# pujariaditya/WaveVerify

Measured on AMD Instinct MI355X. Metric: clips/sec embed+detect, 1s@16kHz bs=256, higher is better.
Workload: dtype f32; 1 GPU; embed_detect: 256 clips x 1 s @ 16 kHz per GPU (BASELINE.json configs[1]), seeded random weights; batch_per_gpu=256, global_batch=256, clip_samples=16000, parallelism=dp1 (independent clip shards, no data-path collective)

## Files before the change

### waveverify_amd/csrc/wv_k1.hip

```cpp
#include <algorithm>
#include <atomic>
#include <cstdlib>
#include <string>
#include <type_traits>

#include "wv_dev.h"

namespace wv {

typedef const __attribute__((address_space(1))) void* gptr_t;
typedef __attribute__((address_space(3))) void* lptr_t;

__device__ __attribute__((aligned(16))) float g_zero16[4] = {0.f, 0.f, 0.f, 0.f};

__device__ __forceinline__ float dpp_next(float v) {
    return __builtin_bit_cast(float, __builtin_amdgcn_update_dpp(0, __builtin_bit_cast(int, v), 0x130, 0xf, 0xf, true));
}

template <int NT_, int BKC_, int BM_ = 128>
struct K1 {
    static constexpr int NT = NT_, BN = 32 * NT_, BKC = BKC_, KQ = BKC_ / 4, BM = BM_, WM = BM_ / 32, NTHREADS = 64 * WM;
    static constexpr int A4 = KQ * BM;
    static constexpr int B4 = BKC * BN / 4;
    static constexpr int STAGE4 = A4 + B4;
    static constexpr int A_PIECES = A4 / 64, B_PIECES = B4 / 64;
    static constexpr int A_PER = (A_PIECES + WM - 1) / WM, B_PER_DMA = (B_PIECES + WM - 1) / WM;
    static constexpr int CG = BN / 4;
    static constexpr int HLD = BN + 4;
    static constexpr int NBT = (BKC / 2) * CG;
    static constexpr int B_PER = (NBT + NTHREADS - 1) / NTHREADS;
    static_assert(A4 % 64 == 0 && B4 % 64 == 0 && NTHREADS % CG == 0 && 64 % CG == 0, "staging maps");
};

template <int NT> struct NVec;
template <> struct NVec<4> { typedef f32x4 type; };
template <> struct NVec<2> { typedef f32x2 type; };

constexpr int OOB_VOFF = 0x40000000;

template <class C>
struct DmaRows {
    const float* src; size_t ld; int K; int rbase;
    __device__ __forceinline__ void init(const float* Xb, int K_, int Tin, int ti0, int wave, int lane) {
        const int col = ti0 + 4 * (lane % C::CG);
        rbase = lane / C::CG;
        const bool inr = col >= 0 && col + 3 < Tin;
        src = inr ? Xb + col : g_zero16;
        ld = inr ? (size_t)Tin : 0;
        K = K_;
        (void)wave;
    }
    __device__ __forceinline__ void init_flat(const float* X, int K_, int Tin, int B, int Tv, int pad, long long g0, int lane) {
        const long long g = g0 + 4 * (lane % C::CG);
        const int b = (int)(g / Tv), t = (int)(g - (long long)b * Tv) - pad;
        rbase = lane / C::CG;
        const bool inr = b < B && t >= 0;
        src = inr ? X + (size_t)b * K_ * Tin + t : g_zero16;
        ld = inr ? (size_t)Tin : 0;
        K = K_;
    }
    __device__ __forceinline__ void issue(int c, f32x4* Bst, int wave) const {
#pragma unroll
        for (int i = 0; i < C::B_PER_DMA; ++i) {
            const int pi = wave + i * C::WM;
            if (C::B_PIECES % C::WM == 0 || pi < C::B_PIECES) {
                const int k = min(c * C::BKC + pi * (64 / C::CG) + rbase, K - 1);
                __builtin_amdgcn_global_load_lds((gptr_t)(src + (size_t)k * ld), (lptr_t)(Bst + pi * 64), 16, 0, 0);
            }
        }
    }
};

template <class C>
struct DmaA {
    __amdgpu_buffer_rsrc_t rsrc;
    int voff[C::A_PER];
    int chunk_bytes;
    __device__ __forceinline__ void init(const f32x4* wq, int Mp, int m0, int nchunks, int wave, int lane) {
        rsrc = __builtin_amdgcn_make_buffer_rsrc(const_cast<f32x4*>(wq + m0), 0, (nchunks * C::KQ * Mp - m0) * 16, 0x00020000);
        chunk_bytes = C::KQ * Mp * 16;
#pragma unroll
        for (int i = 0; i < C::A_PER; ++i) {
            const int idx = (wave + i * C::WM) * 64 + lane;
            voff[i] = ((idx / C::BM) * Mp + idx % C::BM) * 16;
        }
    }
    __device__ __forceinline__ void issue(int c, f32x4* Ast, int wave) const {
        const int soff = c * chunk_bytes;
#pragma unroll
        for (int i = 0; i < C::A_PER; ++i) {
            const int pi = wave + i * C::WM;
            if (C::A_PIECES % C::WM == 0 || pi < C::A_PIECES) {
                const int vo = voff[i];
                __builtin_amdgcn_raw_ptr_buffer_load_lds(rsrc, (lptr_t)(Ast + pi * 64), 16, vo, soff, 0, 0);
            }
        }
    }
};

template <class C, int EPI, int RES>
struct K1Epi {
    static constexpr int NT = C::NT, HLD = C::HLD;
    static constexpr int NTAP = EPI == 0 ? 5 : (EPI == 2 ? 4 : (EPI == 4 ? 8 : 16));
    static constexpr int WLD = EPI == 0 ? 8 : NTAP + 4;
    static constexpr int TABLE_FLOATS = C::BM * WLD;
    static constexpr bool HASR = RES == 1 || RES == 2 || RES == 5;
    static constexpr bool RAWH = RES == 4 || RES == 5;
    static constexpr int RP = HASR ? 4 : 0;
    typedef typename NVec<NT>::type ovec;
    int M, m0, b, to0, lane, wave, half, q, o, to;
    bool act_lane, vec;
    const float* Rb; float* Yb; float* Ab; float* Wl;
    const float* Rb2; float* Hb; float* Sb;
    int voff0, nrec;
    float fgam, fbet;

    __device__ __forceinline__ int row_of(int r) const { return 32 * wave + (r & 3) + 8 * (r >> 2) + 4 * half; }
    __device__ __forceinline__ ovec load_res(const PwDwArgs& p, int r) const {
        ovec v;
#pragma unroll
        for (int e = 0; e < NT; ++e) v[e] = 0.f;
        const int gm = m0 + row_of(r);
        if (act_lane && gm < M) {
            const float* rp = Rb + (size_t)gm * p.Tout + to;
            if (vec) v = *reinterpret_cast<const ovec*>(rp);
            else {
#pragma unroll
                for (int e = 0; e < NT; ++e)
                    if (o + e < p.tto && to + e < p.Tout) v[e] = rp[e];
            }
        }
        return v;
    }
    __device__ __forceinline__ void store(const PwDwArgs& p, int gm, const float (&y)[NT]) const {
        const size_t yo = (size_t)gm * p.Tout + to;
        if (Yb) {
            if (vec) { ovec v; _Pragma("unroll") for (int e = 0; e < NT; ++e) v[e] = y[e]; *reinterpret_cast<ovec*>(Yb + yo) = v; }
            else {
#pragma unroll
                for (int e = 0; e < NT; ++e)
                    if (o + e < p.tto && to + e < p.Tout) Yb[yo + e] = y[e];
            }
        }
        if (Ab) {
            float a[NT];
#pragma unroll
            for (int e = 0; e < NT; ++e) a[e] = elu1(y[e] * p.act_scale);
            if (vec) { ovec v; _Pragma("unroll") for (int e = 0; e < NT; ++e) v[e] = a[e]; *reinterpret_cast<ovec*>(Ab + yo) = v; }
            else {
#pragma unroll
                for (int e = 0; e < NT; ++e)
                    if (o + e < p.tto && to + e < p.Tout) Ab[yo + e] = a[e];
            }
        }
    }
    __device__ __forceinline__ void begin(const PwDwArgs& p, float* table, int m0_, int b_, int to0_, long long gflat = 0) {
        M = p.pw.M; m0 = m0_; b = b_; to0 = to0_;
        const int tid = threadIdx.x;
        lane = tid & 63;
        wave = __builtin_amdgcn_readfirstlane(tid >> 6);
        half = lane >> 5; q = lane & 31;
        Wl = table;
        const size_t bo = (size_t)b * M * p.Tout;
        Yb = p.Y ? p.Y + bo : nullptr;
        Ab = p.Yact ? p.Yact + bo : nullptr;
        Rb = (HASR && p.resid) ? p.resid + bo : nullptr;
        Rb2 = (RES == 2 && p.resid2) ? p.resid2 + bo : nullptr;
        Hb = (RAWH && p.Yraw) ? p.Yraw + bo : nullptr;
        Sb = (RES == 5 && p.Ysum) ? p.Ysum + bo : nullptr;
        o = NT * q; to = to0 + o;
        act_lane = o < p.tto && to < p.Tout;
        vec = act_lane && to + NT - 1 < p.Tout && o + NT - 1 < p.tto && (p.Tout % NT) == 0;
        nrec = M * p.Tout * 4;
        voff0 = act_lane ? ((m0 + 32 * wave + 4 * half) * p.Tout + to) * 4 : 0x7f000000;
        if (EPI == 0 && p.flat) {
            const long long gc = gflat + p.pad + o;
            const int bo2 = (int)(gc / p.Tv), t = (int)(gc - (long long)bo2 * p.Tv) - p.pad;
            const bool ok = o < p.tto && bo2 < p.B && t >= 0;
            Yb = p.Y; Ab = p.Yact; Rb = HASR ? p.resid : nullptr; Rb2 = RES == 2 ? p.resid2 : nullptr; Hb = RAWH ? p.Yraw : nullptr; Sb = RES == 5 ? p.Ysum : nullptr;
            nrec = (int)((long long)p.B * M * p.Tout * 4);
            voff0 = ok ? (int)((((long long)bo2 * M + m0 + 32 * wave + 4 * half) * p.Tout + t) * 4) : (int)0x80000000u;
        }
        if (EPI == 8 && p.flat) {
            const int TvO = p.Tv >> 3;
            const long long go = gflat / 8 + (q >> 1);
            const int bo2 = (int)(go / TvO), n = (int)(go - (long long)bo2 * TvO);
            const bool ok = (q & 1) == 0 && (q >> 1) < p.tto && bo2 < p.B && n < p.Tout;
            Yb = p.Y; Ab = p.Yact;
            nrec = (int)((long long)p.B * M * p.Tout * 4);
            voff0 = ok ? (int)((((long long)bo2 * M + m0 + 32 * wave + 4 * half) * p.Tout + n) * 4) : (int)0x80000000u;
            fgam = 1.f; fbet = 0.f;
            if (p.film) {
                const float* fl = p.film + (size_t)min(bo2, p.B - 1) * p.film_stride + 2 * (m0 / (M / p.bands));
                fgam = fl[0]; fbet = fl[1];
            }
        }
        const bool lane_film = EPI == 8 && p.flat;
        const int bw = p.film ? (M / p.bands) : 1;
        const float* filmb = (p.film && !lane_film) ? p.film + (size_t)b * p.film_stride : nullptr;
        for (int m = tid; m < C::BM; m += C::NTHREADS) {
            const int gm = m0 + m;
            float* row = Wl + m * WLD;
#pragma unroll
            for (int i = 0; i < NTAP; ++i) row[i] = (gm < M && i < p.ks) ? p.dw_w[(size_t)gm * p.ks + i] : 0.f;
            float gam = 1.f, bet = 0.f;
            if (filmb && gm < M) { const int band = gm / bw; gam = filmb[2 * band]; bet = filmb[2 * band + 1]; }
            row[NTAP] = (gm < M && p.dw_b) ? p.dw_b[gm] : 0.f;
            row[NTAP + 1] = gam; row[NTAP + 2] = bet;
            if (EPI != 0) row[WLD - 1] = 0.f;
        }
    }

    typedef unsigned uvec __attribute__((ext_vector_type(NT)));
    __device__ __forceinline__ ovec buf_load(__amdgpu_buffer_rsrc_t r, int off) const {
        if constexpr (NT == 4) return __builtin_bit_cast(ovec, __builtin_amdgcn_raw_buffer_load_b128(r, off, 0, 0));
        else return __builtin_bit_cast(ovec, __builtin_amdgcn_raw_buffer_load_b64(r, off, 0, 0));
    }
    __device__ __forceinline__ void buf_store(__amdgpu_buffer_rsrc_t r, int off, ovec v) const {
        if constexpr (NT == 4) __builtin_amdgcn_raw_buffer_store_b128(__builtin_bit_cast(uvec, v), r, off, 0, 0);
        else __builtin_amdgcn_raw_buffer_store_b64(__builtin_bit_cast(uvec, v), r, off, 0, 0);
    }

    __device__ __forceinline__ void finish(f32x16 (&acc)[NT], const PwDwArgs& p, float* strips) {
        if constexpr (EPI == 0) {
            constexpr int NSH = 4 / NT;
            const int clip_bytes = nrec;
            const __amdgpu_buffer_rsrc_t rY = uniform_rsrc(Yb ? Yb : p.Yact, Yb ? clip_bytes : 0);
            const __amdgpu_buffer_rsrc_t rA = uniform_rsrc(Ab ? Ab : p.Yact, Ab ? clip_bytes : 0);
            const __amdgpu_buffer_rsrc_t rR = uniform_rsrc(Rb ? Rb : p.X, Rb ? clip_bytes : 0);
            const int row_bytes = p.Tout * 4;
            const int voff = voff0;
            const float* Wrow = Wl + (32 * wave + 4 * half) * 8;
            ovec res4[HASR ? 4 : 1];
            ovec add4[RES == 2 ? 4 : 1];
            const __amdgpu_buffer_rsrc_t rR2 = uniform_rsrc(Rb2 ? Rb2 : p.X, Rb2 ? clip_bytes : 0);
            const __amdgpu_buffer_rsrc_t rH = uniform_rsrc(Hb ? Hb : p.Y, Hb ? clip_bytes : 0);
            const __amdgpu_buffer_rsrc_t rS = uniform_rsrc(Sb ? Sb : p.Y, Sb ? clip_bytes : 0);
            const float sres = (RES == 5 && p.scale_ptr) ? p.out_scale * p.scale_ptr[0] : p.out_scale;
            if constexpr (HASR) {
#pragma unroll
                for (int r = 0; r < 4; ++r) res4[r] = buf_load(rR, voff + ((r & 3) + 8 * (r >> 2)) * row_bytes);
            }
            if constexpr (RES == 2) {
#pragma unroll
                for (int r = 0; r < 4; ++r) add4[r] = buf_load(rR2, voff + ((r & 3) + 8 * (r >> 2)) * row_bytes);
            }
            f32x4 w0n = *reinterpret_cast<const f32x4*>(Wrow), w1n = *reinterpret_cast<const f32x4*>(Wrow + 4);
#pragma unroll
            for (int r = 0; r < 16; ++r) {
                const int cr = (r & 3) + 8 * (r >> 2);
                const f32x4 w0 = w0n, w1 = w1n;
                if (r + 1 < 16) {
                    const int cn = ((r + 1) & 3) + 8 * ((r + 1) >> 2);
                    w0n = *reinterpret_cast<const f32x4*>(Wrow + cn * 8);
                    w1n = *reinterpret_cast<const f32x4*>(Wrow + cn * 8 + 4);
                }
                float hh[NT + 4], cur[NT];
#pragma unroll
                for (int e = 0; e < NT; ++e) { cur[e] = acc[e][r]; hh[e] = cur[e]; }
#pragma unroll
                for (int s2 = 1; s2 <= NSH; ++s2) {
#pragma unroll
                    for (int e = 0; e < NT; ++e) { cur[e] = dpp_next(cur[e]); hh[s2 * NT + e] = cur[e]; }
                }
                const int off = voff + cr * row_bytes;
                ovec y;
#pragma unroll
                for (int e = 0; e < NT; ++e) {
                    float v = fmaf(w0.x, hh[e], w1.y);
                    v = fmaf(w0.y, hh[e + 1], v); v = fmaf(w0.z, hh[e + 2], v);
                    v = fmaf(w0.w, hh[e + 3], v); v = fmaf(w1.x, hh[e + 4], v);
                    y[e] = v;
                }
                if constexpr (HASR) {
                    const ovec rr = res4[r & 3];
                    ovec rsum;
                    (void)rsum;
                    if (r + 4 < 16) res4[r & 3] = buf_load(rR, voff + (((r + 4) & 3) + 8 * ((r + 4) >> 2)) * row_bytes);
#pragma unroll
                    for (int e = 0; e < NT; ++e) {
                        if constexpr (RES == 2) {
                            const float z = p.out_scale * rr[e];
                            y[e] = y[e] * (z > 0.f ? 1.f : __expf(z)) * p.out_scale;
                        } else if constexpr (RES == 5) {
                            rsum[e] = fmaf(y[e], sres, rr[e]);
                        } else y[e] = fmaf(y[e], p.out_scale, rr[e]);
                    }
                    if constexpr (RES == 5) buf_store(rS, off, rsum);
                }
                if constexpr (RES == 2) {
                    const ovec ad = add4[r & 3];
                    if (r + 4 < 16) add4[r & 3] = buf_load(rR2, voff + (((r + 4) & 3) + 8 * ((r + 4) >> 2)) * row_bytes);
#pragma unroll
                    for (int e = 0; e < NT; ++e) y[e] += ad[e];
                }
                if constexpr (RAWH) {
                    ovec hraw;
#pragma unroll
                    for (int e = 0; e < NT; ++e) hraw[e] = hh[e + 4];
                    buf_store(rH, off, hraw);
                }
                if (Yb) buf_store(rY, off, y);
                if (Ab) {
                    ovec a;
#pragma unroll
                    for (int e = 0; e < NT; ++e) a[e] = elu1(y[e] * p.act_scale);
                    buf_store(rA, off, a);
                }
                __builtin_amdgcn_sched_barrier(0);
            }
        } else if constexpr (EPI == 5) {
            float* Hw = strips + wave * (4 * HLD);
#pragma unroll
            for (int r = 0; r < 16; ++r) {
                float* strip = Hw + (r & 1) * 2 * HLD;
                ovec hv;
#pragma unroll
                for (int e = 0; e < NT; ++e) hv[e] = acc[e][r];
                *reinterpret_cast<ovec*>(strip + half * HLD + NT * q) = hv;
                const int row = row_of(r), gm = m0 + row;
                const float* wt = Wl + row * WLD;
                const f32x4 ta = *reinterpret_cast<const f32x4*>(wt), tb = *reinterpret_cast<const f32x4*>(wt + 4);
                const f32x4 tc = *reinterpret_cast<const f32x4*>(wt + 8), td = *reinterpret_cast<const f32x4*>(wt + 16);
                if (gm < M && q < p.tto && to0 + q < p.Tout) {
                    const float* hp = strip + half * HLD + p.off + q * 5;
                    float y = td.x;
                    y = fmaf(ta.x, hp[0], y); y = fmaf(ta.y, hp[1], y); y = fmaf(ta.z, hp[2], y); y = fmaf(ta.w, hp[3], y);
                    y = fmaf(tb.x, hp[4], y); y = fmaf(tb.y, hp[5], y); y = fmaf(tb.z, hp[6], y); y = fmaf(tb.w, hp[7], y);
                    y = fmaf(tc.x, hp[8], y); y = fmaf(tc.y, hp[9], y);
                    y = fmaf(y, td.y, td.z);
                    const size_t ro = (size_t)gm * p.Tout + to0 + q;
                    if (Yb) Yb[ro] = y;
                    if (Ab) Ab[ro] = elu1(y * p.act_scale);
                }
            }
        } else if constexpr (EPI >= 2) {
            static_assert(NT == 4 && RES == 0, "strided DPP epilogue: 128-column windows, no residual");
            constexpr int R = EPI;
            const bool flat = R == 8 && p.flat;
            const int clip_bytes = flat ? nrec : M * p.Tout * 4;
            const __amdgpu_buffer_rsrc_t rY = uniform_rsrc(Yb ? Yb : p.Yact, Yb ? clip_bytes : 0);
            const __amdgpu_buffer_rsrc_t rA = uniform_rsrc(Ab ? Ab : p.Yact, Ab ? clip_bytes : 0);
            const int row_bytes = p.Tout * 4;
            const int o0 = R == 2 ? 2 * q : (R == 4 ? q : q >> 1);
            const bool lane_ok = (R != 8 || (q & 1) == 0) && o0 + (R == 2 ? 1 : 0) < p.tto && to0 + o0 + (R == 2 ? 1 : 0) < p.Tout;
            const int voff = flat ? voff0 : (lane_ok ? ((m0 + 32 * wave + 4 * half) * p.Tout + to0 + o0) * 4 : 0x7f000000);
            const float* Wrow = Wl + (32 * wave + 4 * half) * WLD;
#pragma unroll
            for (int r = 0; r < 16; ++r) {
                const int cr = (r & 3) + 8 * (r >> 2);
                constexpr int NL = R == 8 ? 4 : 2;
                float hh[4 * NL], cur[4];
#pragma unroll
                for (int e = 0; e < 4; ++e) { cur[e] = acc[e][r]; hh[e] = cur[e]; }
#pragma unroll
                for (int l = 1; l < NL; ++l) {
#pragma unroll
                    for (int e = 0; e < 4; ++e) { cur[e] = dpp_next(cur[e]); hh[4 * l + e] = cur[e]; }
                }
                const float* wt = Wrow + cr * WLD;
                float w[2 * R];
#pragma unroll
                for (int i = 0; i < 2 * R; i += 4) {
                    const f32x4 v = *reinterpret_cast<const f32x4*>(wt + i);
                    w[i] = v.x; w[i + 1] = v.y; w[i + 2] = v.z; w[i + 3] = v.w;
                }
                const f32x4 bgb = *reinterpret_cast<const f32x4*>(wt + NTAP);
                const int off = voff + cr * row_bytes;
                constexpr int NO = R == 2 ? 2 : 1;
                float y[NO];
#pragma unroll
                for (int j = 0; j < NO; ++j) {
                    const int base = R == 2 ? 2 + 2 * j : 0;
                    float v = bgb.x;
#pragma unroll
                    for (int i = 0; i < 2 * R; ++i) v = fmaf(w[i], hh[base + i], v);
                    y[j] = fmaf(v, bgb.y, bgb.z);
                    if (R == 8 && flat) y[j] = fmaf(y[j], fgam, fbet);
                }
                if constexpr (R == 2) {
                    typedef unsigned u2 __attribute__((ext_vector_type(2)));
                    if (Yb) __builtin_amdgcn_raw_buffer_store_b64(u2{__builtin_bit_cast(unsigned, y[0]), __builtin_bit_cast(unsigned, y[1])}, rY, off, 0, 0);
                    if (Ab) __builtin_amdgcn_raw_buffer_store_b64(u2{__builtin_bit_cast(unsigned, elu1(y[0] * p.act_scale)),
                                                                        __builtin_bit_cast(unsigned, elu1(y[1] * p.act_scale))}, rA, off, 0, 0);
                } else {
                    if (Yb) __builtin_amdgcn_raw_buffer_store_b32(__builtin_bit_cast(unsigned, y[0]), rY, off, 0, 0);
                    if (Ab) __builtin_amdgcn_raw_buffer_store_b32(__builtin_bit_cast(unsigned, elu1(y[0] * p.act_scale)), rA, off, 0, 0);
                }
                __builtin_amdgcn_sched_barrier(0);
            }
        } else {
            float* Hw = strips + wave * (4 * HLD);
            const int ks = p.ks;
            const int no = (p.tto + 31) / 32;
#pragma unroll
            for (int r = 0; r < 16; ++r) {
                float* strip = Hw + (r & 1) * 2 * HLD;
                ovec hv;
#pragma unroll
                for (int e = 0; e < NT; ++e) hv[e] = acc[e][r];
                *reinterpret_cast<ovec*>(strip + half * HLD + NT * q) = hv;
                const int row = row_of(r), gm = m0 + row;
                if (gm >= M) continue;
                const float* wt = Wl + row * WLD;
                const float bias = wt[16], gam = wt[17], bet = wt[18];
                const float* hrow = strip + half * HLD + p.off;
                const size_t ro = (size_t)gm * p.Tout + to0;
                for (int e = 0; e < no; ++e) {
                    const int oo = q * no + e;
                    if (oo >= p.tto || to0 + oo >= p.Tout) break;
                    const float* hp = hrow + oo * p.stride;
                    float y = bias;
                    for (int i = 0; i < ks; ++i) y = fmaf(wt[i], hp[i * p.dil], y);
                    y = fmaf(y, gam, bet);
                    if (RES == 1 && Rb) y = fmaf(y, p.out_scale, Rb[ro + oo]);
                    if (Yb) Yb[ro + oo] = y;
                    if (Ab) Ab[ro + oo] = elu1(y * p.act_scale);
                }
            }
        }
    }
};

template <int LDR> struct LdrSel { typedef RowPairLoader type; };
template <> struct LdrSel<2> { typedef ConvTrPair<4> type; };
template <> struct LdrSel<3> { typedef ConvTrPair<2> type; };
template <> struct LdrSel<4> { typedef ConvTrPair<1> type; };
template <> struct LdrSel<5> { typedef ConvTrPair<0> type; };
template <> struct LdrSel<6> { typedef ConvTrLds<4> type; };
template <> struct LdrSel<7> { typedef ConvTrLds<2> type; };
template <class C> constexpr int k1_lwp(int ldr) { return ldr == 7 ? (C::BN / 2 + 6 + 3) / 4 * 4 : (C::BN / 4 + 6 + 3) / 4 * 4; }

template <class C, int EPI, int LDR, int RES, int NS>
__global__ __launch_bounds__(C::NTHREADS, LDR >= 2 ? (C::B_PER > 1 ? 2 : 3) : 4) void k1_kernel(PwDwArgs p) {
    extern __shared__ __attribute__((aligned(16))) float smem[];
    constexpr bool REG = LDR != 0;
    typedef K1Epi<C, EPI, RES> Epi;
    typedef typename LdrSel<LDR>::type LB;
    typedef typename NVec<C::NT>::type bvec;
    constexpr bool FLAT_OK = EPI == 0 || EPI == 8;
    TileId tile = decode_tile(p);
    if (FLAT_OK && p.flat) {
        const unsigned L = blockIdx.x, j = L >> 3;
        tile.m_tile = j % p.num_m; tile.t_tile = (j / p.num_m) * 8 + (L & 7); tile.b = 0;
        tile.valid = tile.t_tile < p.num_t;
    }
    if (!tile.valid) return;
    const long long gflat = (long long)tile.t_tile * p.tto * p.stride;
    f32x4* S4 = reinterpret_cast<f32x4*>(smem);
    float* table = smem + NS * C::STAGE4 * 4;
    static_assert(NS == 2 || (NS == 3 && LDR == 0), "three stages: DMA path only");
    const int tid = threadIdx.x, lane = tid & 63;
    const int wave = __builtin_amdgcn_readfirstlane(tid >> 6);
    const int h = lane >> 5, i31 = lane & 31;
    const int cg = tid % C::CG;
    const int K = p.pw.K, Mp = p.pw.Mp;
    const int nchunks = (K + C::BKC - 1) / C::BKC;
    const f32x4* wq = reinterpret_cast<const f32x4*>(p.pw.wq);
    const int m0 = tile.m_tile * C::BM, b = tile.b;
    const int to0 = tile.t_tile * p.tto;
    const int ti0 = to0 * p.stride - p.pad - p.off;
    const float* Xb = p.X + (size_t)b * K * p.Tin;

    constexpr int LWP = LDR >= 6 ? k1_lwp<C>(LDR) : 4;
    Epi epi;
    epi.begin(p, table, m0, b, to0, gflat);
    DmaRows<C> db{};
    DmaA<C> da;
    da.init(wq, Mp, m0, nchunks, wave, lane);
    LB lb{};
    float raw[REG ? C::B_PER : 1][REG ? LB::NRAW : 1];
    if constexpr (LDR == 0) {
        if (FLAT_OK && p.flat) db.init_flat(p.X, K, p.Tin, p.B, p.Tv, p.pad, gflat, lane);
        else db.init(Xb, K, p.Tin, ti0, wave, lane);
    }
    else {
        const float* Xt = Xb;
        int c0 = ti0, ncols = p.Tin, tout = p.Tout;
        if (EPI == 0 && p.flat) {
            const long long g = gflat + 4 * cg;
            const int bb = (int)(g / p.Tv), t = (int)(g - (long long)bb * p.Tv) - p.pad;
            const bool inb = bb < p.B;
            Xt = p.X + (size_t)(inb ? bb : 0) * K * p.Tin;
            c0 = t - 4 * cg; ncols = inb ? p.Tin : 0; tout = inb ? p.Tout : 0;
        }
        if constexpr (LDR == 1) lb = LB{Xt, K, p.Tin, ncols, c0, p.pre_scale, p.pre_elu, nullptr, 0, false, false};
        else if constexpr (LDR >= 6) {
            const int lfirst = max(c0, 0) / p.ratio;
            lb = LB{p.ct_w, K, p.ratio, c0, LWP, ((lfirst - 1) & ~3), C::BKC - 1, nullptr, 0, 0};
        }
        else lb = LB{Xt, p.ct_w, p.ct_wt, K, p.pw.Kp, p.Tin, tout, c0, p.ratio, p.pre_scale, p.pre_elu, 0, 0, {}, {}};
    }
    float* Rbuf = table + Epi::TABLE_FLOATS;
    auto issue_rows = [&](int c, int buf) {
        if constexpr (LDR >= 6) {
            constexpr int PPR = LWP / 4, NPIECE = C::BKC * PPR, NINST = (NPIECE + 63) / 64, PER = (NINST + C::WM - 1) / C::WM;
#pragma unroll
            for (int i = 0; i < PER; ++i) {
                const int inst = wave + i * C::WM;
                const int q = inst * 64 + lane;
                const int row = q / PPR, f = lb.ls + 4 * (q - row * PPR);
                const bool inr = f >= 0 && f < p.Tin;
                const float* src = inr ? Xb + (size_t)(c * C::BKC + min(row, C::BKC - 1)) * p.Tin + f : g_zero16;
                if (inst < NINST && q < NPIECE)
                    __builtin_amdgcn_global_load_lds((gptr_t)src, (lptr_t)(Rbuf + (size_t)buf * C::BKC * LWP + inst * 256), 16, 0, 0);
            }
        }
    };

    auto issue = [&](int c, int st) {
        f32x4* S = S4 + st * C::STAGE4;
        da.issue(c, S, wave);
        if constexpr (!REG) db.issue(c, S + C::A4, wave);
    };
    auto fetch = [&](int c) {
        if constexpr (LDR >= 6) { if (c + 1 < nchunks) issue_rows(c + 1, (c + 1) & 1); }
        if constexpr (REG) {
#pragma unroll
            for (int r = 0; r < C::B_PER; ++r) {
                const int idx = tid + r * C::NTHREADS;
                if (C::NBT % C::NTHREADS == 0 || idx < C::NBT) lb.fetch2(c * C::BKC + 2 * (idx / C::CG), raw[r]);
            }
        }
    };
    auto commit = [&](int c, int st) {
        if constexpr (LDR >= 6) lb.Rcur = Rbuf + (size_t)(c & 1) * C::BKC * LWP;
        if constexpr (REG) {
            f32x4* Bq = S4 + st * C::STAGE4 + C::A4;
#pragma unroll
            for (int r = 0; r < C::B_PER; ++r) {
                const int idx = tid + r * C::NTHREADS;
                if (!(C::NBT % C::NTHREADS == 0 || idx < C::NBT)) continue;
                const int kp = idx / C::CG;
                float o[8];
                lb.finish2(c * C::BKC + 2 * kp, raw[r], o);
                Bq[(2 * kp) * C::CG + cg] = f32x4{o[0], o[1], o[2], o[3]};
                Bq[(2 * kp + 1) * C::CG + cg] = f32x4{o[4], o[5], o[6], o[7]};
            }
        }
    };
    constexpr int PIECES_MIN = C::A_PIECES / C::WM + C::B_PIECES / C::WM;
    f32x16 acc[C::NT];
#pragma unroll
    for (int e = 0; e < C::NT; ++e)
#pragma unroll
        for (int r = 0; r < 16; ++r) acc[e][r] = 0.f;
    issue(0, 0);
    if constexpr (NS == 2) {
        if constexpr (LDR >= 6) {
            issue_rows(0, 0);
            __syncthreads();
        }
        if constexpr (REG) { lb.init(cg); fetch(0); commit(0, 0); }
        __syncthreads();
    } else {
        if (nchunks > 1) { issue(1, 1); asm volatile("s_waitcnt vmcnt(%0)" :: "n"(PIECES_MIN) : "memory"); }
        else asm volatile("s_waitcnt vmcnt(0)" ::: "memory");
        asm volatile("s_waitcnt lgkmcnt(0)" ::: "memory");
        __builtin_amdgcn_s_barrier();
    }
    int st = 0;
    for (int c = 0; c < nchunks; ++c) {
        const f32x4* S = S4 + st * C::STAGE4;
        const int stn = st + 1 == NS ? 0 : st + 1;
        if constexpr (NS == 2) {
            if (c + 1 < nchunks) { issue(c + 1, stn); fetch(c + 1); }
        } else {
            if (c + 2 < nchunks) issue(c + 2, stn + 1 == NS ? 0 : stn + 1);
        }
        const float* Bf = reinterpret_cast<const float*>(S + C::A4) + C::NT * i31;
#pragma unroll
        for (int g = 0; g < C::BKC / 16; ++g) {
            const f32x4 a0 = S[(4 * g + h) * C::BM + 32 * wave + i31];
            const f32x4 a1 = S[(4 * g + h + 2) * C::BM + 32 * wave + i31];
#define WV_K1_STEP(AV, ROW)                                                                        \
    { const bvec bv = *reinterpret_cast<const bvec*>(Bf + (ROW) * C::BN);                          \
      _Pragma("unroll") for (int e = 0; e < C::NT; ++e)                                            \
          acc[e] = __builtin_amdgcn_mfma_f32_32x32x2f32(AV, bv[e], acc[e], 0, 0, 0); }
            WV_K1_STEP(a0.x, 16 * g + 4 * h + 0) WV_K1_STEP(a0.y, 16 * g + 4 * h + 1)
            WV_K1_STEP(a0.z, 16 * g + 4 * h + 2) WV_K1_STEP(a0.w, 16 * g + 4 * h + 3)
            WV_K1_STEP(a1.x, 16 * g + 8 + 4 * h + 0) WV_K1_STEP(a1.y, 16 * g + 8 + 4 * h + 1)
            WV_K1_STEP(a1.z, 16 * g + 8 + 4 * h + 2) WV_K1_STEP(a1.w, 16 * g + 8 + 4 * h + 3)
#undef WV_K1_STEP
        }
        if constexpr (NS == 2) {
            if (c + 1 < nchunks) commit(c + 1, stn);
            __syncthreads();
        } else {
            if (c + 2 < nchunks) asm volatile("s_waitcnt vmcnt(%0)" :: "n"(PIECES_MIN) : "memory");
            else asm volatile("s_waitcnt vmcnt(0)" ::: "memory");
            __builtin_amdgcn_s_barrier();
        }
        st = stn;
    }
    epi.finish(acc, p, smem);
}

static bool aligned16(const void* p) { return (reinterpret_cast<uintptr_t>(p) & 15) == 0; }

bool k1_supported(const PwDwArgs& a) {
    if (!a.pw.wq || a.pw.Mp % 128) return false;
    if (a.pw.M < 33) return false;
    if (((a.ct_w ? a.Tout : a.Tin) & 3) || !aligned16(a.X) || a.pw.K < 1) return false;
    if ((long long)a.pw.K * a.Tin * 4 >= OOB_VOFF || (long long)a.pw.M * a.Tout * 4 >= OOB_VOFF) return false;
    if (a.Y && !aligned16(a.Y)) return false;
    if (a.Yact && !aligned16(a.Yact)) return false;
    if (a.resid && !aligned16(a.resid)) return false;
    if ((a.resid2 && !aligned16(a.resid2)) || (a.Yraw && !aligned16(a.Yraw)) || (a.Ysum && !aligned16(a.Ysum))) return false;
    if (a.ks < 1 || a.ks > 16 || (a.ks - 1) * a.dil + 1 + 3 > 64) return false;
    if (a.ct_w && a.ratio == 1) return false;
    return true;
}

template <class C, int EPI, int LDR, int RES, int NS = 2>
static hipError_t k1_run(PwDwArgs a, hipStream_t s, const char* base) {
    const size_t smem = NS * (size_t)C::STAGE4 * 16 + (size_t)K1Epi<C, EPI, RES>::TABLE_FLOATS * sizeof(float) +
                        (LDR >= 6 ? (size_t)2 * C::BKC * k1_lwp<C>(LDR) * sizeof(float) : 0);
    static_assert(C::WM * 4 * C::HLD <= 2 * C::STAGE4 * 4, "strips alias the stages");
    a.num_m = (a.pw.M + C::BM - 1) / C::BM;
    a.num_t = (a.Tout + a.tto - 1) / a.tto;
    a.stagger = 0; a.first_gen = 0;
    long long n_act = (long long)a.num_t * a.B;
    if (a.flat) {
        if (!(C::NT == 4 && (EPI == 0 || (EPI == 8 && LDR == 0)))) return hipErrorInvalidValue;
        n_act = EPI == 8 ? ((long long)a.B * (a.Tv / 8) + a.tto - 1) / a.tto : ((long long)a.B * a.Tv - a.pad + a.tto - 1) / a.tto;
        if (n_act > 0x7fffffffLL) return hipErrorInvalidValue;
        a.num_t = (int)n_act;
    }
    const long long nblk = ((n_act + 7) / 8) * 8 * a.num_m;
    if (nblk > 0x7fffffffLL) return hipErrorInvalidValue;
    std::string name;
    if (prof::enabled())
        name = std::string(base) + "<" + std::to_string(C::BM) + "," + std::to_string(C::BN) + (LDR == 0 ? (NS == 3 ? ",dma3" : ",dma") : (LDR >= 6 ? ",win" : ",reg")) + (a.flat ? ",flat>" : ">");
    const double M = a.pw.M, K = a.pw.K, Bd = a.B;
    const double outs = (a.Y ? 1.0 : 0.0) + (a.Yact ? 1.0 : 0.0) + (a.resid ? 1.0 : 0.0);
    const double flops = a.ct_w ? 2.0 * Bd * a.Tout * K * (M + 2.0) : 2.0 * Bd * M * (K * a.Tin + (double)a.ks * a.Tout);
    prof::Scope ps(s, name.c_str(), flops, 4.0 * Bd * (K * a.Tin + M * a.Tout * outs));
    hipLaunchKernelGGL((k1_kernel<C, EPI, LDR, RES, NS>), dim3((unsigned)nblk), dim3(C::NTHREADS), smem, s, a);
    return hipGetLastError();
}

bool pw_dw_geometry(PwDwArgs& a, int BN);

template <class C, int EPI, int RES>
static hipError_t k1_pick_ldr(const PwDwArgs& a, hipStream_t s) {
    if (a.ct_w) {
        if constexpr (EPI == 0 && RES == 0) {
#ifndef K1_NO_LDS_UPSAMPLE
            if (!a.flat && a.pre_scale == 1.f && !a.pre_elu && a.pw.K % C::BKC == 0 && a.Tin % 4 == 0 && a.Tout == a.Tin * a.ratio && C::BM <= 128) {
                if (a.ratio % 4 == 0) return k1_run<C, 0, 6, false>(a, s, "convtr_pw_lds");
                if (a.ratio == 2) return k1_run<C, 0, 7, false>(a, s, "convtr_pw_lds");
            }
#endif
            if (a.ratio % 4 == 0) return k1_run<C, 0, 2, false>(a, s, "convtr_pw");
            if (a.ratio == 2) return k1_run<C, 0, 3, false>(a, s, "convtr_pw");
            return k1_run<C, 0, 5, false>(a, s, "convtr_pw");
        }
        return hipErrorInvalidValue;
    }
    const char* base = a.spec_add ? "spec_add" : (EPI == 0 ? (RES == 2 ? "pw_dw_k5_dact" : RES == 4 ? "pw_dw_k5_h" : RES == 5 ? "pw_dw_k5_hres" : RES ? "pw_dw_k5" : "pw_dw_k5_nr") : (EPI == 1 ? "pw_dw" : "pw_dw_s"));
    if (a.pre_elu || a.pre_scale != 1.f) return k1_run<C, EPI, 1, RES>(a, s, base);
    if constexpr (C::NT == 4 && C::BM == 128) {
        if (EPI == 0 && a.pw.K >= 256) return k1_run<C, EPI, 0, RES, 3>(a, s, base);
    }
    return k1_run<C, EPI, 0, RES>(a, s, base);
}

template <class C>
static hipError_t k1_pick_epi(const PwDwArgs& a, hipStream_t s, bool k5) {
    const bool res = a.resid != nullptr;
    if (a.res_mode == 2) {
        if (!k5 || !res) return hipErrorNotSupported;
        return k1_pick_ldr<C, 0, 2>(a, s);
    }
    if (a.Yraw) {
        if (!k5 || a.ct_w || (res != (a.Ysum != nullptr))) return hipErrorNotSupported;
        return res ? k1_pick_ldr<C, 0, 5>(a, s) : k1_pick_ldr<C, 0, 4>(a, s);
    }
    if (k5) return res ? k1_pick_ldr<C, 0, true>(a, s) : k1_pick_ldr<C, 0, false>(a, s);
    if constexpr (C::NT == 4) {
        if (!res && !a.ct_w && a.dil == 1 && a.ks == 2 * a.stride && a.pad == a.stride &&
            a.off == (a.stride == 2 ? 2 : 0)) {
            if (a.stride == 2) return k1_pick_ldr<C, 2, false>(a, s);
            if (a.stride == 4) return k1_pick_ldr<C, 4, false>(a, s);
            if (a.stride == 8) return k1_pick_ldr<C, 8, false>(a, s);
        }
        if (!res && !a.ct_w && a.dil == 1 && a.ks == 10 && a.stride == 5 && a.tto <= 32) return k1_pick_ldr<C, 5, false>(a, s);
    }
    return res ? k1_pick_ldr<C, 1, true>(a, s) : k1_pick_ldr<C, 1, false>(a, s);
}

hipError_t launch_k1(const PwDwArgs& a0, hipStream_t s) {
    PwDwArgs a = a0;
    const bool k5 = a.ks == 5 && a.stride == 1 && a.dil == 1 && a.pad == 4 && !a.film;
    const int need = (a.ks - 1) * a.dil + 1;
    bool narrow = (a.ct_w ? a.Tout : a.Tin) + a.pad + 3 <= 64;
    if (!narrow) {
        PwDwArgs g128 = a, g64 = a;
        if (pw_dw_geometry(g128, 128) && pw_dw_geometry(g64, 64)) {
            const long long c128 = (long long)((a.Tout + g128.tto - 1) / g128.tto) * 128;
            const long long c64 = (long long)((a.Tout + g64.tto - 1) / g64.tto) * 64;
            if (c64 * 100 < c128 * 95) narrow = true;
        }
    }
    (void)need;
    a.flat = 0;
    if (k5 && a.B > 1 && (a.Tout & 3) == 0) {
        int bm = 128, best = (a.pw.M + 127) / 128 * 128;
        for (int cand : {96, 64}) { const int pd = (a.pw.M + cand - 1) / cand * cand; if (pd < best) { best = pd; bm = cand; } }
        const long long Tv = a.Tout + 4;
        const long long flat_cols = ((long long)a.B * Tv - 4 + 123) / 124 * 128;
        PwDwArgs g = a;
        const int bn = narrow ? 64 : 128;
        long long clip_cols = -1;
        if (pw_dw_geometry(g, bn)) clip_cols = (long long)a.B * ((a.Tout + g.tto - 1) / g.tto) * bn;
        if (a.pw.M % bm == 0 && (long long)a.B * a.pw.M * a.Tout * 4 < 0x7fffffffLL && clip_cols > 0 &&
            flat_cols * 100 < clip_cols * 98) {
            a.flat = 1; a.Tv = (int)Tv; narrow = false;
        }
    }
    if (!pw_dw_geometry(a, narrow ? 64 : 128)) return hipErrorNotSupported;
    if (!narrow && !a.flat && !a.resid && !a.ct_w && a.ks == 16 && a.stride == 8 && a.dil == 1 && a.pad == 8 && a.off == 0 && a.B > 1 &&
        a.Tin % 8 == 0 && a.Tout * 8 == a.Tin && a.pw.M % 128 == 0 && (!a.film || (a.pw.M / a.bands) % 128 == 0) && !a.pre_elu && a.pre_scale == 1.f &&
        (long long)a.B * a.pw.M * a.Tout * 4 < 0x7fffffffLL && (long long)a.B * a.pw.K * a.Tin * 4 < 0x7fffffffLL) {
        const long long flat_tiles = ((long long)a.B * ((a.Tin + 8) / 8) + a.tto - 1) / a.tto;
        const long long clip_tiles = (long long)a.B * ((a.Tout + a.tto - 1) / a.tto);
        if (flat_tiles * 100 < clip_tiles * 98) { a.flat = 1; a.Tv = a.Tin + 8; }
    }
    if ((a.tto * a.stride) % 4 != 0 || (a.pad + a.off) % 4 != 0) return hipErrorNotSupported;
    int bm = 128, best = (a.pw.M + 127) / 128 * 128;
    for (int cand : {96, 64}) {
        const int padded = (a.pw.M + cand - 1) / cand * cand;
        if (padded < best) { best = padded; bm = cand; }
    }
    if (narrow) {
        if (bm == 128) return k1_pick_epi<K1<2, 32, 128>>(a, s, k5);
        if (bm == 96) return k1_pick_epi<K1<2, 32, 96>>(a, s, k5);
        return k1_pick_epi<K1<2, 32, 64>>(a, s, k5);
    }
    if (a.ct_w && k5 && !narrow && !a.resid && !a.Yraw && a.res_mode != 2 && a.pw.M % 256 == 0) return k1_pick_ldr<K1<4, 16, 256>, 0, false>(a, s);
    if (bm == 128) return k1_pick_epi<K1<4, 16, 128>>(a, s, k5);
    if (bm == 96) return k1_pick_epi<K1<4, 16, 96>>(a, s, k5);
    return k1_pick_epi<K1<4, 16, 64>>(a, s, k5);
}


template <class C, bool FUSE>
__global__ __launch_bounds__(C::NTHREADS, (FUSE && C::BM == 64) ? 2 : ((FUSE || C::B_PER > 1) ? 3 : 4)) void stft_k1_kernel(StftArgs p, SpecAddArgs q) {
    constexpr bool PRE_RES = FUSE && C::BM == 64;
    extern __shared__ __attribute__((aligned(16))) float smem[];
    typedef typename NVec<C::NT>::type bvec;
    typedef unsigned uvec __attribute__((ext_vector_type(C::NT)));
    const unsigned L = blockIdx.x, j = L >> 3;
    const int m_tile = j % p.num_m;
    const unsigned n_idx = (j / p.num_m) * 8 + (L & 7);
    if (n_idx >= (unsigned)p.num_t * p.B) return;
    const int t_tile = n_idx % p.num_t, b = n_idx / p.num_t;
    f32x4* S4 = reinterpret_cast<f32x4*>(smem);
    const int tid = threadIdx.x, lane = tid & 63;
    const int wave = __builtin_amdgcn_readfirstlane(tid >> 6);
    const int h = lane >> 5, i31 = lane & 31, cg = tid % C::CG;
    const int K = p.n_fft, m0 = m_tile * C::BM, t0 = t_tile * C::BN;
    const int nchunks = (K + C::BKC - 1) / C::BKC;
    const float* wb = p.wav + (size_t)b * p.T;
    DmaA<C> da;
    da.init(reinterpret_cast<const f32x4*>(p.basis_q), p.Mp, m0, nchunks, wave, lane);

    int sbase[4]; bool fv[4];
#pragma unroll
    for (int e = 0; e < 4; ++e) {
        const int t = t0 + 4 * cg + e;
        fv[e] = t < p.Tf;
        sbase[e] = t * p.hop - (p.n_fft - 1);
    }
    const bool interior = (K % C::BKC) == 0 && t0 + C::BN <= p.Tf && (long long)t0 * p.hop - (p.n_fft - 1) >= 0 &&
                          (long long)(t0 + C::BN - 1) * p.hop < p.T;
    float raw[C::B_PER][8];
    const bool side_on = m_tile == 0;
    float d0[4] = {0.f, 0.f, 0.f, 0.f}, d1[4] = {0.f, 0.f, 0.f, 0.f};
    auto fetch = [&](int c, auto FAST) {
#pragma unroll
        for (int r = 0; r < C::B_PER; ++r) {
            const int idx = tid + r * C::NTHREADS;
            if (!(C::NBT % C::NTHREADS == 0 || idx < C::NBT)) continue;
            const int k0 = c * C::BKC + 2 * (idx / C::CG);
            if constexpr (decltype(FAST)::value) {
#pragma unroll
                for (int e = 0; e < 4; ++e) {
                    const f32x2u v = *reinterpret_cast<const f32x2u*>(wb + (sbase[e] + k0));
                    raw[r][e] = v.x; raw[r][4 + e] = v.y;
                }
            } else {
#pragma unroll
                for (int i = 0; i < 2; ++i)
#pragma unroll
                    for (int e = 0; e < 4; ++e) raw[r][4 * i + e] = wb[min(max(sbase[e] + k0 + i, 0), p.T - 1)];
            }
        }
    };
    auto commit = [&](int c, int st, auto FAST) {
        f32x4* Bq = S4 + st * C::STAGE4 + C::A4;
#pragma unroll
        for (int r = 0; r < C::B_PER; ++r) {
            const int idx = tid + r * C::NTHREADS;
            if (!(C::NBT % C::NTHREADS == 0 || idx < C::NBT)) continue;
            const int kp = idx / C::CG, k0 = c * C::BKC + 2 * kp;
            float o[8];
#pragma unroll
            for (int i = 0; i < 2; ++i)
#pragma unroll
                for (int e = 0; e < 4; ++e) {
                    if constexpr (decltype(FAST)::value) o[4 * i + e] = raw[r][4 * i + e];
                    else {
                        const int sidx = sbase[e] + k0 + i;
                        o[4 * i + e] = (fv[e] && k0 + i < K && sidx >= 0 && sidx < p.T) ? raw[r][4 * i + e] : 0.f;
                    }
                }
            Bq[(2 * kp) * C::CG + cg] = f32x4{o[0], o[1], o[2], o[3]};
            Bq[(2 * kp + 1) * C::CG + cg] = f32x4{o[4], o[5], o[6], o[7]};
            if (side_on) {
#pragma unroll
                for (int i = 0; i < 2; ++i) {
                    const int k = min(k0 + i, K - 1);
                    const float s0 = p.side[k], s1 = p.side[K + k];
#pragma unroll
                    for (int e = 0; e < 4; ++e) { d0[e] = fmaf(s0, o[4 * i + e], d0[e]); d1[e] = fmaf(s1, o[4 * i + e], d1[e]); }
                }
            }
        }
    };
    f32x16 acc[C::NT];
#pragma unroll
    for (int e = 0; e < C::NT; ++e)
#pragma unroll
        for (int r = 0; r < 16; ++r) acc[e][r] = 0.f;
    auto gemm = [&](auto FAST) {
        da.issue(0, S4, wave);
        fetch(0, FAST); commit(0, 0, FAST);
        __syncthreads();
        for (int c = 0; c < nchunks; ++c) {
            const int st = c & 1;
            const f32x4* S = S4 + st * C::STAGE4;
            if (c + 1 < nchunks) { da.issue(c + 1, S4 + (st ^ 1) * C::STAGE4, wave); fetch(c + 1, FAST); }
            const float* Bf = reinterpret_cast<const float*>(S + C::A4) + C::NT * i31;
#pragma unroll
            for (int g = 0; g < C::BKC / 16; ++g) {
                const f32x4 a0 = S[(4 * g + h) * C::BM + 32 * wave + i31];
                const f32x4 a1 = S[(4 * g + h + 2) * C::BM + 32 * wave + i31];
#define WV_ST_STEP(AV, ROW)                                                                        \
    { const bvec bv = *reinterpret_cast<const bvec*>(Bf + (ROW) * C::BN);                          \
      _Pragma("unroll") for (int e = 0; e < C::NT; ++e)                                            \
          acc[e] = __builtin_amdgcn_mfma_f32_32x32x2f32(AV, bv[e], acc[e], 0, 0, 0); }
                WV_ST_STEP(a0.x, 16 * g + 4 * h + 0) WV_ST_STEP(a0.y, 16 * g + 4 * h + 1)
                WV_ST_STEP(a0.z, 16 * g + 4 * h + 2) WV_ST_STEP(a0.w, 16 * g + 4 * h + 3)
                WV_ST_STEP(a1.x, 16 * g + 8 + 4 * h + 0) WV_ST_STEP(a1.y, 16 * g + 8 + 4 * h + 1)
                WV_ST_STEP(a1.z, 16 * g + 8 + 4 * h + 2) WV_ST_STEP(a1.w, 16 * g + 8 + 4 * h + 3)
#undef WV_ST_STEP
            }
            if (c + 1 < nchunks) commit(c + 1, st ^ 1, FAST);
            __syncthreads();
        }
    };
    if (interior) gemm(std::true_type{});
    else gemm(std::false_type{});
    float* sd = smem;
    if (side_on) {
        const int slot = tid / C::CG;
#pragma unroll
        for (int e = 0; e < 4; ++e) {
            sd[(slot * C::BN + 4 * cg + e) * 2] = d0[e];
            sd[(slot * C::BN + 4 * cg + e) * 2 + 1] = d1[e];
        }
        __syncthreads();
    }
    constexpr int NSLOT = C::NTHREADS / C::CG;
    const int clip_bytes = p.F * p.Tf * 4;
    const __amdgpu_buffer_rsrc_t rP = uniform_rsrc(FUSE ? p.wav : p.P + (size_t)b * p.F * p.Tf, FUSE ? 0 : clip_bytes);
    const int tq = t0 + C::NT * i31;
    const bool lane_ok = tq < p.Tf;
    auto logmag = [&](float re, float im) { return stft_logmag(re, im, p.c1, p.c0); };
    constexpr int F16 = FUSE ? (C::BM / 2 + 1 + 15) / 16 * 16 : 0, NC2 = F16 / 16;
    float* Pl = smem + NSLOT * C::BN * 2;
    f32x4 a2[FUSE ? NC2 : 1][2];
    if constexpr (FUSE) {
        const __amdgpu_buffer_rsrc_t rW = uniform_rsrc(q.pw.wq, NC2 * 4 * q.pw.Mp * 16);
        const int avoff = (h * q.pw.Mp + 32 * wave + i31) * 16;
#pragma unroll
        for (int c = 0; c < NC2; ++c) {
            a2[c][0] = __builtin_bit_cast(f32x4, __builtin_amdgcn_raw_buffer_load_b128(rW, avoff, c * 4 * q.pw.Mp * 16, 0));
            a2[c][1] = __builtin_bit_cast(f32x4, __builtin_amdgcn_raw_buffer_load_b128(rW, avoff, (c * 4 + 2) * q.pw.Mp * 16, 0));
        }
        for (int i = tid; i < (F16 - (C::BM / 2 + 1)) * C::BN; i += C::NTHREADS) Pl[(C::BM / 2 + 1) * C::BN + i] = 0.f;
    }
#pragma unroll
    for (int r = 0; r < 16; r += 2) {
        const int row = m0 + 32 * wave + (r & 3) + 8 * (r >> 2) + 4 * h;
        const bool row_ok = lane_ok && row < p.n_fft;
        if (row == 0) {
            bvec y0, y1;
#pragma unroll
            for (int e = 0; e < C::NT; ++e) {
                float s0 = 0.f, s1 = 0.f;
                const int col = C::NT * i31 + e;
                for (int sl = 0; sl < NSLOT; ++sl) { s0 += sd[(sl * C::BN + col) * 2]; s1 += sd[(sl * C::BN + col) * 2 + 1]; }
                y0[e] = logmag(acc[e][r], s0);
                y1[e] = logmag(acc[e][r + 1], s1);
            }
            if constexpr (FUSE) {
                *reinterpret_cast<bvec*>(Pl + C::NT * i31) = y0;
                *reinterpret_cast<bvec*>(Pl + (p.F - 1) * C::BN + C::NT * i31) = y1;
            } else {
                const int v0 = lane_ok ? tq * 4 : 0x7f000000, v1 = lane_ok ? ((p.F - 1) * p.Tf + tq) * 4 : 0x7f000000;
                if constexpr (C::NT == 4) {
                    __builtin_amdgcn_raw_buffer_store_b128(__builtin_bit_cast(uvec, y0), rP, v0, 0, 0);
                    __builtin_amdgcn_raw_buffer_store_b128(__builtin_bit_cast(uvec, y1), rP, v1, 0, 0);
                } else {
                    __builtin_amdgcn_raw_buffer_store_b64(__builtin_bit_cast(uvec, y0), rP, v0, 0, 0);
                    __builtin_amdgcn_raw_buffer_store_b64(__builtin_bit_cast(uvec, y1), rP, v1, 0, 0);
                }
            }
        } else {
            bvec y;
#pragma unroll
            for (int e = 0; e < C::NT; ++e) y[e] = logmag(acc[e][r], acc[e][r + 1]);
            if constexpr (FUSE) {
                *reinterpret_cast<bvec*>(Pl + (row >> 1) * C::BN + C::NT * i31) = y;
            } else {
                const int v = row_ok ? ((row >> 1) * p.Tf + tq) * 4 : 0x7f000000;
                if constexpr (C::NT == 4) __builtin_amdgcn_raw_buffer_store_b128(__builtin_bit_cast(uvec, y), rP, v, 0, 0);
                else __builtin_amdgcn_raw_buffer_store_b64(__builtin_bit_cast(uvec, y), rP, v, 0, 0);
            }
        }
    }
    if constexpr (FUSE) {
        bvec resA[PRE_RES ? 16 : 1];
        if constexpr (PRE_RES) {
            const int M_ = C::BM, blk_ = M_ * p.Tf * 4;
            const __amdgpu_buffer_rsrc_t rR_ = uniform_rsrc(q.resid + (size_t)b * M_ * p.Tf, blk_);
            const int voff_ = lane_ok ? ((32 * wave + 4 * h) * p.Tf + tq) * 4 : 0x7f000000;
#pragma unroll
            for (int r = 0; r < 16; ++r) {
                const int o_ = voff_ + ((r & 3) + 8 * (r >> 2)) * p.Tf * 4;
                if constexpr (C::NT == 4) resA[r] = __builtin_bit_cast(bvec, __builtin_amdgcn_raw_buffer_load_b128(rR_, o_, 0, 0));
                else resA[r] = __builtin_bit_cast(bvec, __builtin_amdgcn_raw_buffer_load_b64(rR_, o_, 0, 0));
            }
        }
        __syncthreads();
#pragma unroll
        for (int e = 0; e < C::NT; ++e)
#pragma unroll
            for (int r = 0; r < 16; ++r) acc[e][r] = 0.f;
        const float* Bf = Pl + C::NT * i31 + 4 * h * C::BN;
#pragma unroll
        for (int c = 0; c < NC2; ++c) {
#pragma unroll
            for (int j = 0; j < 8; ++j) {
                const bvec bv = *reinterpret_cast<const bvec*>(Bf + (16 * c + (j < 4 ? j : 4 + j)) * C::BN);
                const float a = a2[c][j >> 2][j & 3];
#pragma unroll
                for (int e = 0; e < C::NT; ++e) acc[e] = __builtin_amdgcn_mfma_f32_32x32x2f32(a, bv[e], acc[e], 0, 0, 0);
            }
        }
        const int M = C::BM, blk = M * p.Tf * 4;
        const size_t bo = (size_t)b * M * p.Tf;
        const __amdgpu_buffer_rsrc_t rR = uniform_rsrc(q.resid + bo, blk);
        const __amdgpu_buffer_rsrc_t rY = uniform_rsrc(q.Y ? q.Y + bo : q.resid, q.Y ? blk : 0);
// ... 89 lines not shown
```

Measured before the change: 3495 clips/s.

## Load GEMM A-operand weights straight into registers in the three-stage K1 loop

For the 3-stage DMA pointwise-conv path (K>=256, RES 0/1 except K=512 residual), weight tiles now come from global memory into VGPRs through inline buffer_load_dwordx4, one chunk ahead. They no longer go through LDS with buffer_load_lds. This shrinks the LDS stage footprint and drops the LDS reads of A in the inner loop. The cost is more VGPR pressure, hand-written inline asm with manual waitcnt coupling, and a loop unrolled by two with register ping-pong.

Result: no change. 3469 clips/s (-0.7%).

```diff
diff --git a/waveverify_amd/csrc/wv_k1.hip b/waveverify_amd/csrc/wv_k1.hip
--- a/waveverify_amd/csrc/wv_k1.hip
+++ b/waveverify_amd/csrc/wv_k1.hip
@@ -96,6 +96,33 @@
             }
         }
     }
+};
+
+template <class C>
+struct RegA {
+    typedef unsigned u32x4 __attribute__((ext_vector_type(4)));
+    u32x4 rsrc;
+    int voff, chunk_bytes, row2_bytes;
+    __device__ __forceinline__ void init(const f32x4* wq, int Mp, int m0, int nchunks, int wave, int lane) {
+        const unsigned long long base = reinterpret_cast<unsigned long long>(wq + m0);
+        rsrc = u32x4{(unsigned)__builtin_amdgcn_readfirstlane((int)(unsigned)base), (unsigned)__builtin_amdgcn_readfirstlane((int)(unsigned)(base >> 32)) & 0xffffu,
+                     (unsigned)__builtin_amdgcn_readfirstlane((nchunks * C::KQ * Mp - m0) * 16), 0x00020000u};
+        chunk_bytes = C::KQ * Mp * 16; row2_bytes = 2 * Mp * 16;
+        voff = ((lane >> 5) * Mp + 32 * wave + (lane & 31)) * 16;
+    }
+    __device__ __forceinline__ void load(int c, f32x4 (&dst)[2]) const {
+        const int so = __builtin_amdgcn_readfirstlane(c * chunk_bytes), so2 = __builtin_amdgcn_readfirstlane(c * chunk_bytes + row2_bytes);
+        asm volatile("s_nop 4\n\tbuffer_load_dwordx4 %0, %2, %3, %4 offen\n\tbuffer_load_dwordx4 %1, %2, %3, %5 offen"
+                     : "=&v"(dst[0]), "=&v"(dst[1]) : "v"(voff), "s"(rsrc), "s"(so), "s"(so2) : "memory");
+    }
+    __device__ __forceinline__ static void acquire(f32x4 (&a)[2]) { asm volatile("" : "+v"(a[0]), "+v"(a[1]) :: "memory"); }
+};
+
+template <class C, bool AR>
+struct K1Stage {
+    static constexpr int A4 = AR ? 0 : C::A4;
+    static constexpr int STAGE4 = A4 + C::B4;
+    static constexpr int PIECES_MIN = (AR ? 0 : C::A_PIECES / C::WM) + C::B_PIECES / C::WM;
 };
 
 template <class C, int EPI, int RES>
@@ -431,10 +458,12 @@
 template <> struct LdrSel<7> { typedef ConvTrLds<2> type; };
 template <class C> constexpr int k1_lwp(int ldr) { return ldr == 7 ? (C::BN / 2 + 6 + 3) / 4 * 4 : (C::BN / 4 + 6 + 3) / 4 * 4; }
 
-template <class C, int EPI, int LDR, int RES, int NS>
+template <class C, int EPI, int LDR, int RES, int NS, bool AR>
 __global__ __launch_bounds__(C::NTHREADS, LDR >= 2 ? (C::B_PER > 1 ? 2 : 3) : 4) void k1_kernel(PwDwArgs p) {
     extern __shared__ __attribute__((aligned(16))) float smem[];
     constexpr bool REG = LDR != 0;
+    typedef K1Stage<C, AR> Stg;
+    static_assert(!AR || (NS == 3 && LDR == 0 && C::BKC == 16), "register A: the three-stage DMA loop, one 16-deep group per chunk");
     typedef K1Epi<C, EPI, RES> Epi;
     typedef typename LdrSel<LDR>::type LB;
     typedef typename NVec<C::NT>::type bvec;
@@ -448,7 +477,7 @@
     if (!tile.valid) return;
     const long long gflat = (long long)tile.t_tile * p.tto * p.stride;
     f32x4* S4 = reinterpret_cast<f32x4*>(smem);
-    float* table = smem + NS * C::STAGE4 * 4;
+    float* table = smem + NS * Stg::STAGE4 * 4;
     static_assert(NS == 2 || (NS == 3 && LDR == 0), "three stages: DMA path only");
     const int tid = threadIdx.x, lane = tid & 63;
     const int wave = __builtin_amdgcn_readfirstlane(tid >> 6);
@@ -467,7 +496,9 @@
     epi.begin(p, table, m0, b, to0, gflat);
     DmaRows<C> db{};
     DmaA<C> da;
-    da.init(wq, Mp, m0, nchunks, wave, lane);
+    RegA<C> wa;
+    if constexpr (AR) wa.init(wq, Mp, m0, nchunks, wave, lane);
+    else da.init(wq, Mp, m0, nchunks, wave, lane);
     LB lb{};
     float raw[REG ? C::B_PER : 1][REG ? LB::NRAW : 1];
     if constexpr (LDR == 0) {
@@ -509,9 +540,9 @@
     };
 
     auto issue = [&](int c, int st) {
-        f32x4* S = S4 + st * C::STAGE4;
-        da.issue(c, S, wave);
-        if constexpr (!REG) db.issue(c, S + C::A4, wave);
+        f32x4* S = S4 + st * Stg::STAGE4;
+        if constexpr (!AR) da.issue(c, S, wave);
+        if constexpr (!REG) db.issue(c, S + Stg::A4, wave);
     };
     auto fetch = [&](int c) {
         if constexpr (LDR >= 6) { if (c + 1 < nchunks) issue_rows(c + 1, (c + 1) & 1); }
@@ -526,7 +557,7 @@
     auto commit = [&](int c, int st) {
         if constexpr (LDR >= 6) lb.Rcur = Rbuf + (size_t)(c & 1) * C::BKC * LWP;
         if constexpr (REG) {
-            f32x4* Bq = S4 + st * C::STAGE4 + C::A4;
+            f32x4* Bq = S4 + st * Stg::STAGE4 + Stg::A4;
 #pragma unroll
             for (int r = 0; r < C::B_PER; ++r) {
                 const int idx = tid + r * C::NTHREADS;
@@ -539,12 +570,14 @@
             }
         }
     };
-    constexpr int PIECES_MIN = C::A_PIECES / C::WM + C::B_PIECES / C::WM;
+    constexpr int PIECES_MIN = Stg::PIECES_MIN;
+    f32x4 ra[2], rb[2];
     f32x16 acc[C::NT];
 #pragma unroll
     for (int e = 0; e < C::NT; ++e)
 #pragma unroll
         for (int r = 0; r < 16; ++r) acc[e][r] = 0.f;
+    if constexpr (AR) wa.load(0, ra);
     issue(0, 0);
     if constexpr (NS == 2) {
         if constexpr (LDR >= 6) {
@@ -556,23 +589,30 @@
     } else {
         if (nchunks > 1) { issue(1, 1); asm volatile("s_waitcnt vmcnt(%0)" :: "n"(PIECES_MIN) : "memory"); }
         else asm volatile("s_waitcnt vmcnt(0)" ::: "memory");
+        if constexpr (AR) RegA<C>::acquire(ra);
         asm volatile("s_waitcnt lgkmcnt(0)" ::: "memory");
         __builtin_amdgcn_s_barrier();
     }
     int st = 0;
-    for (int c = 0; c < nchunks; ++c) {
-        const f32x4* S = S4 + st * C::STAGE4;
+    auto chunk = [&](int c, const f32x4 (&cur)[2], f32x4 (&nxt)[2]) {
+        const f32x4* S = S4 + st * Stg::STAGE4;
         const int stn = st + 1 == NS ? 0 : st + 1;
+        if constexpr (AR) wa.load(min(c + 1, nchunks - 1), nxt);
         if constexpr (NS == 2) {
             if (c + 1 < nchunks) { issue(c + 1, stn); fetch(c + 1); }
         } else {
             if (c + 2 < nchunks) issue(c + 2, stn + 1 == NS ? 0 : stn + 1);
         }
-        const float* Bf = reinterpret_cast<const float*>(S + C::A4) + C::NT * i31;
+        if constexpr (AR) __builtin_amdgcn_sched_barrier(0);
+        const float* Bf = reinterpret_cast<const float*>(S + Stg::A4) + C::NT * i31;
 #pragma unroll
         for (int g = 0; g < C::BKC / 16; ++g) {
-            const f32x4 a0 = S[(4 * g + h) * C::BM + 32 * wave + i31];
-            const f32x4 a1 = S[(4 * g + h + 2) * C::BM + 32 * wave + i31];
+            f32x4 a0, a1;
+            if constexpr (AR) { a0 = cur[0]; a1 = cur[1]; }
+            else {
+                a0 = S[(4 * g + h) * C::BM + 32 * wave + i31];
+                a1 = S[(4 * g + h + 2) * C::BM + 32 * wave + i31];
+            }
 #define WV_K1_STEP(AV, ROW)                                                                        \
     { const bvec bv = *reinterpret_cast<const bvec*>(Bf + (ROW) * C::BN);                          \
       _Pragma("unroll") for (int e = 0; e < C::NT; ++e)                                            \
@@ -589,9 +629,18 @@
         } else {
             if (c + 2 < nchunks) asm volatile("s_waitcnt vmcnt(%0)" :: "n"(PIECES_MIN) : "memory");
             else asm volatile("s_waitcnt vmcnt(0)" ::: "memory");
+            if constexpr (AR) RegA<C>::acquire(nxt);
             __builtin_amdgcn_s_barrier();
         }
         st = stn;
+    };
+    if constexpr (AR) {
+        for (int c = 0; c < nchunks; c += 2) {
+            chunk(c, ra, rb);
+            if (c + 1 < nchunks) chunk(c + 1, rb, ra);
+        }
+    } else {
+        for (int c = 0; c < nchunks; ++c) chunk(c, ra, rb);
     }
     epi.finish(acc, p, smem);
 }
@@ -612,11 +661,12 @@
     return true;
 }
 
-template <class C, int EPI, int LDR, int RES, int NS = 2>
+template <class C, int EPI, int LDR, int RES, int NS = 2, bool AR = false>
 static hipError_t k1_run(PwDwArgs a, hipStream_t s, const char* base) {
-    const size_t smem = NS * (size_t)C::STAGE4 * 16 + (size_t)K1Epi<C, EPI, RES>::TABLE_FLOATS * sizeof(float) +
+    typedef K1Stage<C, AR> Stg;
+    const size_t smem = NS * (size_t)Stg::STAGE4 * 16 + (size_t)K1Epi<C, EPI, RES>::TABLE_FLOATS * sizeof(float) +
                         (LDR >= 6 ? (size_t)2 * C::BKC * k1_lwp<C>(LDR) * sizeof(float) : 0);
-    static_assert(C::WM * 4 * C::HLD <= 2 * C::STAGE4 * 4, "strips alias the stages");
+    static_assert(C::WM * 4 * C::HLD <= 2 * Stg::STAGE4 * 4, "strips alias the stages");
     a.num_m = (a.pw.M + C::BM - 1) / C::BM;
     a.num_t = (a.Tout + a.tto - 1) / a.tto;
     a.stagger = 0; a.first_gen = 0;
@@ -636,7 +686,7 @@
     const double outs = (a.Y ? 1.0 : 0.0) + (a.Yact ? 1.0 : 0.0) + (a.resid ? 1.0 : 0.0);
     const double flops = a.ct_w ? 2.0 * Bd * a.Tout * K * (M + 2.0) : 2.0 * Bd * M * (K * a.Tin + (double)a.ks * a.Tout);
     prof::Scope ps(s, name.c_str(), flops, 4.0 * Bd * (K * a.Tin + M * a.Tout * outs));
-    hipLaunchKernelGGL((k1_kernel<C, EPI, LDR, RES, NS>), dim3((unsigned)nblk), dim3(C::NTHREADS), smem, s, a);
+    hipLaunchKernelGGL((k1_kernel<C, EPI, LDR, RES, NS, AR>), dim3((unsigned)nblk), dim3(C::NTHREADS), smem, s, a);
     return hipGetLastError();
 }
 
@@ -661,7 +711,12 @@
     const char* base = a.spec_add ? "spec_add" : (EPI == 0 ? (RES == 2 ? "pw_dw_k5_dact" : RES == 4 ? "pw_dw_k5_h" : RES == 5 ? "pw_dw_k5_hres" : RES ? "pw_dw_k5" : "pw_dw_k5_nr") : (EPI == 1 ? "pw_dw" : "pw_dw_s"));
     if (a.pre_elu || a.pre_scale != 1.f) return k1_run<C, EPI, 1, RES>(a, s, base);
     if constexpr (C::NT == 4 && C::BM == 128) {
-        if (EPI == 0 && a.pw.K >= 256) return k1_run<C, EPI, 0, RES, 3>(a, s, base);
+        if constexpr (EPI == 0) {
+            if (a.pw.K >= 256) {
+                if constexpr (RES == 0 || RES == 1) { if (!(RES == 1 && a.pw.K == 512)) return k1_run<C, EPI, 0, RES, 3, true>(a, s, base); }
+                return k1_run<C, EPI, 0, RES, 3>(a, s, base);
+            }
+        }
     }
     return k1_run<C, EPI, 0, RES>(a, s, base);
 }
```
